# codybloemhard/termdaw

Measured on AMD Instinct MI355X. Metric: offline render Msamples/sec (stereo 48 kHz) + % HBM roofline, 64-vertex graph, higher is better.
Workload: dtype f32; 1 GPU; BASELINE config 2: 64 sampleloop -> 1 normalize, 60 s @48 kHz, bl 1024, 16-bit PCM out; 1 project(s) per GPU per step (project p of the job on rank p mod N, seed offset 64*p); frames_per_project=2880512, projects_per_gpu=1, vertices_per_project=65, normalize=one launch, output=int16 PCM in HBM, parallelism=project p on rank p mod N; one RCCL all-reduce(max) of the 1-entry peak table

## Files before the change

### termdaw_amd/csrc/engine.cpp

```cpp
#include <chrono>

#include "engine.h"
#include "chorus_math.h"
#include "comm.h"
#include "compile.h"
#include "delay_math.h"
#include "devmem.h"
#include "eq_math.h"
#include "midi.h"
#include "sat_math.h"

#include <math.h>
#include <stdlib.h>
#include <string.h>

#include <algorithm>
#include <map>
#include <tuple>
#include <mutex>
#include <condition_variable>
#include <atomic>
#include <thread>
#include <limits>

// ... 242 lines not shown
    const size_t nmax = std::max(nl, nr);
    float *d_lin = nullptr, *d_l = nullptr, *d_r = nullptr, *d_s = nullptr;
    uint8_t* d_raw = nullptr;
    auto cleanup = [&]() {};
    {
        auto up = [](size_t b) { return (b + 255) & ~(size_t)255; };
        const size_t bps_raw = linear ? 0 : (raw_format == PCM_U8 ? 1 : raw_format == PCM_S16 ? 2 : raw_format == PCM_S24 ? 3 : 4);
        const size_t b_lin = up(std::max<size_t>(n_values, 1) * sizeof(float)), b_ch = up(std::max<size_t>(nmax, 1) * sizeof(float));
        const size_t b_raw = up(std::max<size_t>(n_values * bps_raw, 1));
        const size_t need = b_lin + 2 * b_ch + 256 + b_raw;
        if (need > sb->tmp_cap) {
            TD_HIP(hipDeviceSynchronize());
            if (sb->tmp) (void)hipFree(sb->tmp);
            sb->tmp = nullptr;
            sb->tmp_cap = 0;
            TD_HIP(hipMalloc(&sb->tmp, need + need / 2));
            sb->tmp_cap = need + need / 2;
        }
        unsigned char* p = sb->tmp;
        d_lin = reinterpret_cast<float*>(p); p += b_lin;
        d_l = reinterpret_cast<float*>(p); p += b_ch;
        d_r = reinterpret_cast<float*>(p); p += b_ch;
        d_s = reinterpret_cast<float*>(p); p += 256;
        d_raw = p;
    }
    if (linear) {
        TD_HIP(hipMemcpyAsync(d_lin, linear, n_values * sizeof(float), hipMemcpyHostToDevice, st));
    } else {
        const size_t bps = raw_format == PCM_U8 ? 1 : raw_format == PCM_S16 ? 2 : raw_format == PCM_S24 ? 3 : 4;
        TD_HIP(hipMemcpyAsync(d_raw, raw, n_values * bps, hipMemcpyHostToDevice, st));
        launch_pcm_decode(d_raw, d_lin, (uint32_t)n_values, raw_format, st);
    }
    if (pick_loudest) {
        if (channels == 1) {
            launch_sample_split(d_lin, 1, 0, 0, d_l, d_r, (uint32_t)nl, (uint32_t)nr, st);
        } else {
            launch_sample_split(d_lin, 2, 0, 1, d_l, d_r, (uint32_t)nl, (uint32_t)nr, st);
        }
        launch_abs_sum_serial(d_l, (uint32_t)nl, d_s + 4, st);
        launch_abs_sum_serial(d_r, (uint32_t)nr, d_s + 5, st);
        float sums[2];
        TD_HIP(hipMemcpyAsync(sums, d_s + 4, 8, hipMemcpyDeviceToHost, st));
        TD_HIP(hipStreamSynchronize(st));
        const float lm = nl ? sums[0] / (float)nl : 0.0f, rm = nr ? sums[1] / (float)nr : 0.0f;
        const bool take_l = lm > rm;
        const size_t n_take = take_l ? nl : nr;
        if (n_take == 0) { cleanup(); return fail("termdaw_amd: loudest channel is empty"); }
        TD_HIP(hipMemcpyAsync(take_l ? d_r : d_l, take_l ? d_l : d_r, n_take * sizeof(float), hipMemcpyDeviceToDevice, st));
        nl = nr = n_take;
    } else {
        launch_sample_split(d_lin, (uint32_t)channels, src_l, src_r, d_l, d_r, (uint32_t)nl, (uint32_t)nr, st);
    }
    size_t n = nl;
    const float *p_max_l = d_s, *p_max_r = d_s + 1;
    if (method == LM_NORM) {
        launch_absmax(d_l, (uint32_t)nl, d_s, st);
        launch_absmax(d_r, (uint32_t)nr, d_s + 1, st);
    } else if (method == LM_MIX) {
        n = std::min(nl, nr);
        launch_add_planar(d_l, d_r, d_l, (uint32_t)n, st);
        launch_absmax(d_l, (uint32_t)n, d_s, st);
        TD_HIP(hipMemcpyAsync(d_r, d_l, n * sizeof(float), hipMemcpyDeviceToDevice, st));
        p_max_r = d_s;
    } else {
        launch_absmax(d_l, (uint32_t)nl, d_s, st);
        launch_absmax(d_r, (uint32_t)nr, d_s + 1, st);
        launch_absmax(d_s, 2, d_s + 2, st);
        p_max_l = p_max_r = d_s + 2;
    }
    if (nl != nr && method != LM_MIX) { cleanup(); return fail("termdaw_amd: channel lengths differ after load"); }
    if (n == 0) { cleanup(); return fail("TermDaw: Sample::from: l and r have length 0."); }
    SampleEntry e;
    e.len = n;
    e.d = static_cast<float2*>(sb->alloc(0, (n + 16 + (n & 1)) * sizeof(float2)));
    if (!e.d) return 0;
    struct Guard {
        td_samplebank* sb; SampleEntry* e; bool armed = true;
        ~Guard() { if (armed) { sb->release(e->d); sb->release(e->d16); } }
    } guard{sb, &e};
    TD_HIP(hipMemsetAsync(e.d + n, 0, (16 + (n & 1)) * sizeof(float2), st));
    launch_sample_pack(d_l, d_r, p_max_l, p_max_r, e.d, (uint32_t)n, st);
    bool want16 = method != LM_MIX && sr == sb->sample_rate && n >= 1 && n < 0x3FFFFFF0u;
    if (want16) {
        e.d16 = static_cast<uint32_t*>(sb->alloc(1, ((n + 18) & ~(size_t)3) * sizeof(uint32_t)));
        if (!e.d16) return 0;
        TD_HIP(hipMemsetAsync(d_s + 8, 0, sizeof(uint32_t), st));
        launch_sample_pack16(d_l, d_r, e.d16, (uint32_t)n, reinterpret_cast<uint32_t*>(d_s + 8), st);
    }
    float host_s[12] = {0};
    TD_HIP(hipMemcpyAsync(host_s, d_s, sizeof host_s, hipMemcpyDeviceToHost, st));
    TD_HIP(hipStreamSynchronize(st));
    TD_HIP(hipGetLastError());
    if (want16) {
        uint32_t bad;
        memcpy(&bad, &host_s[8], 4);
        const float ml = host_s[p_max_l - d_s], mr = host_s[p_max_r - d_s];
        if (bad) {
            sb->release(e.d16);
            e.d16 = nullptr;
        } else {
            e.scale_l = 1.0f / ml;
            e.scale_r = 1.0f / mr;
        }
    }
    cleanup();
    if (sr != sb->sample_rate) {
        float2* rs = nullptr;
        size_t nout = 0;
        if (!resample_device(e.d, e.len, sr, sb->sample_rate, &rs, &nout, st)) return 0;
        sb->release(e.d);
        e.d = rs;
        if (nout == 0) return fail("termdaw_amd: resampled sample is empty");
        e.len = nout;
    }
    guard.armed = false;
    sb->samples.push_back(e);
    sb->names[name] = sb->samples.size() - 1;
    return 1;
}

}

using namespace tde;

uint64_t td_flowwbank::next_version() {
    static std::atomic<uint64_t> counter{1};
    return counter.fetch_add(1);
}
void td_flowwbank::set_start_indices_to_frame(size_t t_frame, bool do_skip) {
    for (size_t i = 0; i < flowws.size(); ++i) {
        const auto& fl = flowws[i];
        for (size_t j = do_skip ? start_indices[i] : 0; j < fl.size(); ++j) {
            if (frame_of(fl[j]) >= t_frame) {
                start_indices[i] = j;
                break;
            }
        }
    }
}
void td_flowwbank::set_time(size_t t) {
    set_start_indices_to_frame(t, false);
    frame = t;
}
void td_flowwbank::set_time_to_next_block() {
    frame += bl;
    set_start_indices_to_frame(frame, true);
}

namespace tde {
int upload_tables(td_graph* g, TableCache& tc, const Staging& tmp) {
    const size_t bytes = std::max<size_t>(tmp.b.size(), 16);
    if (bytes > tc.cap) {
        TD_HIP(hipStreamSynchronize(g->stream));
        if (tc.d) { (void)hipFree(tc.d); g->device_bytes -= tc.cap; }
        if (tc.h) (void)hipHostFree(tc.h);
        tc.d = tc.h = nullptr;
        tc.cap = 0;
        tc.inflight = false;
        const size_t cap = bytes + bytes / 4 + 256;
        TD_HIP(hipMalloc(&tc.d, cap));
        TD_HIP(hipHostMalloc(&tc.h, cap, hipHostMallocDefault));
        if (!tc.copied) TD_HIP(hipEventCreateWithFlags(&tc.copied, hipEventDisableTiming));
        tc.cap = cap;
        g->device_bytes += cap;
    }
    if (tc.inflight) TD_HIP(hipEventSynchronize(tc.copied));
    tc.inflight = false;
// ... 2710 lines not shown
```

### termdaw_amd/csrc/kernels.h

```cpp
#pragma once
#include <hip/hip_runtime.h>
#include <stdint.h>
#include "adsr_math.h"

namespace tdk {

constexpr int kThreads = 256;
constexpr int kTileFrames = 1024;
constexpr uint32_t kBandMaxSegs = 131072;
constexpr uint32_t kBandMaxS = 1024;

struct PanGain {
    float l_amp, r_amp, gain;
    uint32_t flags;
};

struct InTerm {
    const float2* p;
    uint64_t len;
    uint64_t t0;
    PanGain pg;
    uint32_t kind;
    uint32_t magic;
    float scale_l, scale_r;
};
enum TermMode : uint32_t { TERMS_MIXED = 0, TERMS_ALL_EDGE = 1, TERMS_ALL_LOOP32 = 2, TERMS_ALL_LOOP16 = 3,
                           TERMS_EDGE_FEW = 4,
                           TERMS_ADSR1 = 5,
                           TERMS_WITH_ADSR = 6 };

struct NormState { float max, scan_max; uint32_t violated, ticket; };

struct BandRespParam {
    double ql[8], qh[8];
    double gl, gh;
    double* resp;
};

struct SumDesc {
    const InTerm* ins;
    float2* out;
    float* peaks;
    const NormState* state;
    float* init_copy;
    float init_max;
    uint32_t use_init;
    uint32_t k;
    uint32_t mode;
    uint32_t term_mode;
    uint32_t debug;
    PanGain pg;
    float2* out_q4;
    void* pcm;
    float amplitude;
    uint32_t qmode;
    const BandRespParam* rp;
    unsigned long long* sync;
    uint32_t* host_flag;
};

struct ScaleDesc {
    float2* buf;
    const float* peaks;
    const float* init_copy;
    NormState* state;
    void* pcm;
    float amplitude;
    uint32_t qmode;
    PanGain pg;
    uint32_t pcm_only;
    uint32_t pad[3];
};

struct QuantDesc {
    const float2* in;
    void* pcm;
    float amplitude;
    uint32_t qmode;
};

struct StemDesc {
    InTerm src;
    void* pcm;
    float2* f32;
    uint32_t* peak;
    float amplitude;
    uint32_t qmode;
};

struct LoudDesc {
    const void* pcm;
// ... 470 lines not shown
```

### termdaw_amd/csrc/kernels.hip

```cpp
#include "kernels.h"

#include <algorithm>

namespace tdk {

#define TD_DEV __device__ __forceinline__

TD_DEV float2 epilogue(float2 v, const PanGain& pg) {
    if (pg.flags & 1u) { v.x *= pg.l_amp; v.y *= pg.r_amp; }
    if (pg.flags & 2u) { v.x *= pg.gain;  v.y *= pg.gain;  }
    return v;
}
TD_DEV float4 epilogue4(float4 v, const PanGain& pg) {
    float2 a = epilogue(make_float2(v.x, v.y), pg), b = epilogue(make_float2(v.z, v.w), pg);
    return make_float4(a.x, a.y, b.x, b.y);
}

#define TD_GLOBAL __attribute__((address_space(1)))
typedef float f4v __attribute__((ext_vector_type(4)));
typedef float f2v __attribute__((ext_vector_type(2)));
typedef unsigned int u2v __attribute__((ext_vector_type(2)));
typedef int i4v __attribute__((ext_vector_type(4)));
typedef int i2v __attribute__((ext_vector_type(2)));
TD_DEV float4 gload4(const void* p) { const f4v v = *reinterpret_cast<const f4v TD_GLOBAL*>((const TD_GLOBAL char*)p); return make_float4(v.x, v.y, v.z, v.w); }
// ... 250 lines not shown
#pragma unroll
            for (int u = 0; u < 4; ++u) { const float2* p = ins[j + 4 + u].p; b0[u] = load_pair(p, m0, M); b1[u] = load_pair(p, m1, M); }
#pragma unroll
            for (int u = 0; u < 4; ++u) { acc0 = add4(acc0, a0[u]); acc1 = add4(acc1, a1[u]); }
            if (j + 12 <= k) {
#pragma unroll
                for (int u = 0; u < 4; ++u) { const float2* p = ins[j + 8 + u].p; a0[u] = load_pair(p, m0, M); a1[u] = load_pair(p, m1, M); }
            }
#pragma unroll
            for (int u = 0; u < 4; ++u) { acc0 = add4(acc0, b0[u]); acc1 = add4(acc1, b1[u]); }
        }
        if (j + 4 <= k) {
#pragma unroll
            for (int u = 0; u < 4; ++u) { acc0 = add4(acc0, a0[u]); acc1 = add4(acc1, a1[u]); }
            j += 4;
        }
    }
    for (; j + 4 <= k; j += 4) {
        float4 x0[4], x1[4];
#pragma unroll
        for (int u = 0; u < 4; ++u) {
            if (MODE == TERMS_ALL_EDGE || MODE == TERMS_EDGE_FEW) { const float2* p = ins[j + u].p; x0[u] = load_pair(p, m0, M); x1[u] = load_pair(p, m1, M); }
            else if (MODE == TERMS_ALL_LOOP32) { x0[u] = loop_term_pair(ins, j + u, m0, M); x1[u] = loop_term_pair(ins, j + u, m1, M); }
            else { x0[u] = term_pair(ins, j + u, m0, M); x1[u] = term_pair(ins, j + u, m1, M); }
        }
#pragma unroll
        for (int u = 0; u < 4; ++u) { acc0 = add4(acc0, x0[u]); acc1 = add4(acc1, x1[u]); }
    }
    for (; j < k; ++j) {
        acc0 = add4(acc0, term_pair(ins, j, m0, M));
        acc1 = add4(acc1, term_pair(ins, j, m1, M));
    }
}
typedef unsigned int u4v __attribute__((ext_vector_type(4)));
TD_DEV float2 unpack16(uint32_t w, float sl, float sr) {
    return make_float2((float)(int16_t)(w & 0xFFFFu) * sl, (float)(int16_t)(w >> 16) * sr);
}
typedef unsigned int u4v_u __attribute__((ext_vector_type(4), aligned(4)));
TD_DEV void loop16_quad(const uint32_t* s, uint32_t len, uint32_t idx, uint32_t out[4]) {
    (void)len;
    const uint32_t TD_GLOBAL* g = reinterpret_cast<const uint32_t TD_GLOBAL*>((const TD_GLOBAL char*)s);
    const u4v_u q = *reinterpret_cast<const u4v_u TD_GLOBAL*>(g + idx);
    out[0] = q.x; out[1] = q.y; out[2] = q.z; out[3] = q.w;
}
TD_DEV f2v cvt16(uint32_t w) { f2v v; v.x = (float)(int16_t)(w & 0xFFFFu); v.y = (float)(int16_t)(w >> 16); return v; }
TD_DEV void sum_terms16(TermTab ins, uint32_t k, uint32_t m, uint32_t M, float4& acc0, float4& acc1) {
    f2v c[4];
#pragma unroll
    for (int f = 0; f < 4; ++f) { c[f].x = 0.f; c[f].y = 0.f; }
    auto add_term = [&](uint32_t j, const uint32_t w[4]) {
        f2v sc, am, gn;
        sc.x = ins[j].scale_l; sc.y = ins[j].scale_r;
        am.x = ins[j].pg.l_amp; am.y = ins[j].pg.r_amp;
        gn.x = gn.y = ins[j].pg.gain;
#pragma unroll
        for (int f = 0; f < 4; ++f) {
            f2v v = cvt16(w[f]) * sc;
            v = v * am;
            v = v * gn;
            c[f] = c[f] + v;
        }
    };
    auto gather = [&](uint32_t j, uint32_t w[4]) {
        const uint32_t len = (uint32_t)ins[j].len;
        loop16_quad(reinterpret_cast<const uint32_t*>(ins[j].p), len, barrett_mod((uint32_t)ins[j].t0 + m, len, ins[j].magic), w);
    };
    uint32_t j = 0;
    for (; j + 4 <= k; j += 4) {
        uint32_t w[4][4];
#pragma unroll
        for (int u = 0; u < 4; ++u) gather(j + u, w[u]);
#pragma unroll
        for (int u = 0; u < 4; ++u) add_term(j + u, w[u]);
    }
    for (; j < k; ++j) {
        uint32_t w[4];
        gather(j, w);
        add_term(j, w);
    }
    acc0 = zero_tail(make_float4(c[0].x, c[0].y, c[1].x, c[1].y), m, M);
    acc1 = zero_tail(make_float4(c[2].x, c[2].y, c[3].x, c[3].y), m + 2u, M);
}

TD_DEV uint32_t step256(uint32_t len, uint32_t magic) {
    const uint32_t r = 256u - __umulhi(256u, magic) * len;
    return r >= len ? r - len : r;
}
template <int NQ>
TD_DEV uint32_t quad_frame(uint32_t m, int q) { return NQ == 4 ? m + 256u * (uint32_t)q : m + 4u * (uint32_t)q; }
template <int NQ>
TD_DEV uint32_t pair_frame(uint32_t m, int p) { return quad_frame<NQ>(m, p >> 1) + 2u * (uint32_t)(p & 1); }
template <int NQ>
TD_DEV void sum_terms16w(TermTab ins, uint32_t k, uint32_t m, uint32_t M, float4 acc[2 * NQ]) {
    f2v c[4 * NQ];
#pragma unroll
    for (int f = 0; f < 4 * NQ; ++f) { c[f].x = 0.f; c[f].y = 0.f; }
    auto add_term = [&](uint32_t j, const uint32_t w[4 * NQ]) {
        f2v sc, am, gn;
        sc.x = ins[j].scale_l; sc.y = ins[j].scale_r;
        am.x = ins[j].pg.l_amp; am.y = ins[j].pg.r_amp;
        gn.x = gn.y = ins[j].pg.gain;
#pragma unroll
        for (int f = 0; f < 4 * NQ; ++f) {
            f2v v = cvt16(w[f]) * sc;
            v = v * am;
            v = v * gn;
            c[f] = c[f] + v;
        }
    };
    auto gather = [&](uint32_t j, uint32_t w[4 * NQ]) {
        const uint32_t len = (uint32_t)ins[j].len;
        const uint32_t idx = barrett_mod((uint32_t)ins[j].t0 + m, len, ins[j].magic);
        if (NQ == 4) {
            const uint32_t* p = reinterpret_cast<const uint32_t*>(ins[j].p);
            const uint32_t step = step256(len, ins[j].magic);
            uint32_t i = idx;
#pragma unroll
            for (int q = 0; q < NQ; ++q) {
                loop16_quad(p, len, i, w + 4 * q);
                i += step;
                i = min(i, i - len);
            }
            return;
        }
#pragma unroll
        for (int q = 0; q < NQ; ++q) loop16_quad(reinterpret_cast<const uint32_t*>(ins[j].p), len, idx + 4u * q, w + 4 * q);
    };
    uint32_t j = 0;
    constexpr int B = 4;
    for (; j + B <= k; j += B) {
        uint32_t w[B][4 * NQ];
#pragma unroll
        for (int u = 0; u < B; ++u) gather(j + u, w[u]);
#pragma unroll
        for (int u = 0; u < B; ++u) add_term(j + u, w[u]);
    }
    for (; j < k; ++j) { uint32_t w[4 * NQ]; gather(j, w); add_term(j, w); }
#pragma unroll
    for (int q = 0; q < 2 * NQ; ++q) acc[q] = zero_tail(make_float4(c[2 * q].x, c[2 * q].y, c[2 * q + 1].x, c[2 * q + 1].y), pair_frame<NQ>(m, q), M);
}

template <int NQ>
TD_DEV void sum_terms32w(TermTab ins, uint32_t k, uint32_t m, uint32_t M, float4 acc[2 * NQ]) {
    f4v c[2 * NQ];
#pragma unroll
    for (int q = 0; q < 2 * NQ; ++q) { c[q].x = 0.f; c[q].y = 0.f; c[q].z = 0.f; c[q].w = 0.f; }
    constexpr int B = NQ >= 4 ? 1 : 2;
    auto gather = [&](uint32_t j, f4v x[2 * NQ]) {
        const uint32_t len = (uint32_t)ins[j].len;
        const uint32_t idx = barrett_mod((uint32_t)ins[j].t0 + m, len, ins[j].magic);
        const float2* p = ins[j].p + idx;
#pragma unroll
        for (int q = 0; q < 2 * NQ; ++q) {
            const float4 v = gload4u(p + 2 * q);
            x[q].x = v.x; x[q].y = v.y; x[q].z = v.z; x[q].w = v.w;
        }
    };
    auto add_term = [&](uint32_t j, const f4v x[2 * NQ]) {
        f4v am, gn;
        am.x = am.z = ins[j].pg.l_amp; am.y = am.w = ins[j].pg.r_amp;
        gn.x = gn.y = gn.z = gn.w = ins[j].pg.gain;
#pragma unroll
        for (int q = 0; q < 2 * NQ; ++q) {
            f4v v = x[q] * am;
            v = v * gn;
            c[q] = c[q] + v;
        }
    };
    uint32_t j = 0;
    for (; j + B <= k; j += B) {
        f4v x[B][2 * NQ];
#pragma unroll
        for (int u = 0; u < B; ++u) gather(j + u, x[u]);
#pragma unroll
        for (int u = 0; u < B; ++u) add_term(j + u, x[u]);
    }
    for (; j < k; ++j) { f4v x[2 * NQ]; gather(j, x); add_term(j, x); }
#pragma unroll
    for (int q = 0; q < 2 * NQ; ++q) acc[q] = zero_tail(make_float4(c[q].x, c[q].y, c[q].z, c[q].w), m + 2u * q, M);
}

TD_DEV void sum_inputs_pairs(const InTerm* ins_generic, uint32_t k, uint32_t term_mode, uint32_t m0, uint32_t m1, uint32_t M,
                             float4& a0, float4& a1) {
    const TermTab ins = term_tab(ins_generic);
    a0 = make_float4(0.f, 0.f, 0.f, 0.f);
    a1 = a0;
    if (term_mode == TERMS_ALL_EDGE) sum_terms<TERMS_ALL_EDGE>(ins, k, m0, m1, M, a0, a1);
    else if (term_mode == TERMS_ALL_LOOP32) sum_terms<TERMS_ALL_LOOP32>(ins, k, m0, m1, M, a0, a1);
    else if (term_mode == TERMS_ADSR1) sum_terms<TERMS_ADSR1>(ins, k, m0, m1, M, a0, a1);
    else if (term_mode == TERMS_WITH_ADSR) sum_terms<TERMS_WITH_ADSR>(ins, k, m0, m1, M, a0, a1);
    else sum_terms<TERMS_MIXED>(ins, k, m0, m1, M, a0, a1);
}

TD_DEV float absmax4(float m, float4 v) {
    m = fmaxf(m, fabsf(v.x)); m = fmaxf(m, fabsf(v.y));
    m = fmaxf(m, fabsf(v.z)); m = fmaxf(m, fabsf(v.w));
    return m;
}

template <int TMODE>
__global__ __launch_bounds__(kThreads) void k_sum(const SumDesc* __restrict__ descs, uint32_t M, uint32_t bl,
                                                  uint32_t tiles_per_block) {
    const SumDesc& d = descs[blockIdx.y];
    constexpr bool quad_map = TMODE == TERMS_ALL_LOOP16;
    const uint32_t m0 = blockIdx.x * kTileFrames + (quad_map ? 4 : 2) * threadIdx.x;
    const uint32_t m1 = m0 + (quad_map ? 2 : kTileFrames / 2);
    float4 a0 = make_float4(0.f, 0.f, 0.f, 0.f), a1 = a0;
    if (quad_map) sum_terms16(term_tab(d.ins), d.k, m0, M, a0, a1);
    else sum_terms<TMODE>(term_tab(d.ins), d.k, m0, m1, M, a0, a1);
    if (d.mode == 0) {
        store_pair(d.out, m0, M, epilogue4(a0, d.pg));
        store_pair(d.out, m1, M, epilogue4(a1, d.pg));
        return;
    }
    float spec_init = 0.0f;
    if (d.mode == 3) {
        spec_init = d.use_init ? d.init_max : d.state->max;
        const float r = 1.0f / spec_init;
        const float4 s0 = epilogue4(make_float4(a0.x * r, a0.y * r, a0.z * r, a0.w * r), d.pg);
        const float4 s1 = epilogue4(make_float4(a1.x * r, a1.y * r, a1.z * r, a1.w * r), d.pg);
        if (d.out) {
            store_pair(d.out, m0, M, s0);
// ... 55 lines not shown
            if ((threadIdx.x & 63u) == 63u) {
#pragma unroll
                for (int e = 0; e < 8; ++e) if (!((e & 2) ? want_h : want_l)) rh[e][threadIdx.x >> 6] = 0.0;
            }
            __syncthreads();
            if (threadIdx.x < 16u) {
                const uint32_t blk_in_tile = threadIdx.x >> 2, chain = threadIdx.x & 3u;
                const uint32_t q0 = (blk_in_tile & 1u) * 2u, e = (blk_in_tile >> 1) * 4u + chain;
                const uint32_t blk = blockIdx.x * 4u + blk_in_tile;
                if (blk * 256u < M) rp.resp[4u * blk + chain] = rh[e][q0] + rh[e][q0 + 1u];
            }
        }
        __shared__ float bp[kThreads / 64][2];
        __shared__ uint32_t bc[kThreads / 64][2];
        __shared__ float2 first[4];
        if ((threadIdx.x & 127) == 0) {
            first[(threadIdx.x >> 7)] = make_float2(a0.x, a0.y);
            first[2 + (threadIdx.x >> 7)] = make_float2(a1.x, a1.y);
        }
        __syncthreads();
        const float2 f0 = first[threadIdx.x >> 7], f1 = first[2 + (threadIdx.x >> 7)];
        auto same2 = [](float4 a, float2 f) {
            return __float_as_uint(a.x) == __float_as_uint(f.x) && __float_as_uint(a.y) == __float_as_uint(f.y) &&
                   __float_as_uint(a.z) == __float_as_uint(f.x) && __float_as_uint(a.w) == __float_as_uint(f.y);
        };
        float p0 = m0 < M ? absmax4(0.0f, a0) : 0.0f, p1 = m1 < M ? absmax4(0.0f, a1) : 0.0f;
        const bool c0 = __all((m0 + 1 >= M || same2(a0, f0)) ? 1 : 0) != 0, c1 = __all((m1 + 1 >= M || same2(a1, f1)) ? 1 : 0) != 0;
        p0 = wave_max(p0);
        p1 = wave_max(p1);
        if ((threadIdx.x & 63) == 0) {
            bp[threadIdx.x >> 6][0] = p0; bp[threadIdx.x >> 6][1] = p1;
            bc[threadIdx.x >> 6][0] = c0; bc[threadIdx.x >> 6][1] = c1;
        }
        __syncthreads();
        if (threadIdx.x < 4) {
            const uint32_t half = threadIdx.x & 1u, pair = threadIdx.x >> 1;
            const uint32_t blk = blockIdx.x * 4u + pair * 2u + half;
            const bool cst = bc[2 * half][pair] && bc[2 * half + 1][pair];
            if (blk * 256u < M) d.peaks[blk] = cst ? -1.0f : fmaxf(bp[2 * half][pair], bp[2 * half + 1][pair]);
        }
        return;
    }
    if (blockIdx.x == 0 && threadIdx.x == 0) {
        d.init_copy[0] = d.use_init ? d.init_max : d.state->max;
        d.init_copy[1] = d.state->scan_max;
    }
    const bool spec = d.mode == 3;
    if (tiles_per_block) {
        float pk = 0.0f;
        if (m0 < M) pk = absmax4(pk, a0);
        if (m1 < M) pk = absmax4(pk, a1);
        pk = wave_max(pk);
        __shared__ float wmax[kThreads / 64];
        if ((threadIdx.x & 63) == 0) wmax[threadIdx.x >> 6] = pk;
        __syncthreads();
        if (threadIdx.x == 0) {
            pk = fmaxf(fmaxf(wmax[0], wmax[1]), fmaxf(wmax[2], wmax[3]));
            uint32_t b = blockIdx.x / tiles_per_block;
            if (tiles_per_block == 1) d.peaks[b] = pk;
            else atomicMax(reinterpret_cast<unsigned int*>(d.peaks + b), __float_as_uint(pk));
            if (spec && pk > spec_init) const_cast<NormState*>(d.state)->violated = 1u;
        }
    } else {
        if (spec) {
            const float pk = fmaxf(m0 < M ? absmax4(0.0f, a0) : 0.0f, m1 < M ? absmax4(0.0f, a1) : 0.0f);
            if (pk > spec_init) const_cast<NormState*>(d.state)->violated = 1u;
        }
        const float v[8] = {a0.x, a0.y, a0.z, a0.w, a1.x, a1.y, a1.z, a1.w};
#pragma unroll
        for (int f = 0; f < 4; ++f) {
            uint32_t m = (f < 2 ? m0 : m1) + (f & 1);
            if (m < M) {
                float pk = fmaxf(fmaxf(0.0f, fabsf(v[2 * f])), fabsf(v[2 * f + 1]));
                atomicMax(reinterpret_cast<unsigned int*>(d.peaks + m / bl), __float_as_uint(pk));
            }
        }
    }
}

template <int NQ, bool PACKED = true>
__global__ __launch_bounds__(kThreads) void k_sum16w(const SumDesc* __restrict__ descs, uint32_t M, uint32_t tag) {
    const SumDesc& d = descs[blockIdx.y];
    constexpr int SH = (NQ == 4 && PACKED) ? 4 : 1;
    const uint32_t m = SH == 4 ? blockIdx.x * (kTileFrames * NQ) + (threadIdx.x >> 6) * kTileFrames + 4u * (threadIdx.x & 63u)
                               : blockIdx.x * (kTileFrames * NQ) + 4u * NQ * threadIdx.x;
    const float spec_init_early = d.mode >= 4 ? (d.use_init ? d.init_max : gload1(&d.state->max)) : 0.0f;
    float4 a[2 * NQ];
    if (PACKED) sum_terms16w<NQ>(term_tab(d.ins), d.k, m, M, a);
    else sum_terms32w<NQ>(term_tab(d.ins), d.k, m, M, a);
    if (d.mode == 0) {
#pragma unroll
        for (int q = 0; q < 2 * NQ; ++q) store_pair(d.out, pair_frame<SH>(m, q), M, epilogue4(a[q], d.pg));
        return;
    }
    float pk = 0.0f;
#pragma unroll
    for (int q = 0; q < 2 * NQ; ++q) if (pair_frame<SH>(m, q) < M) pk = absmax4(pk, a[q]);
    float spec_init = 0.0f;
    if (d.mode >= 4) {
        const float init = spec_init_early;
        __shared__ float wm4[kThreads / 64], pm4[kThreads / 64];
        __shared__ uint32_t bad4;
        const uint32_t wave = threadIdx.x >> 6;
        const float pw = wave_max(pk);
        if ((threadIdx.x & 63) == 0) wm4[wave] = pw;
        if (threadIdx.x == 0) bad4 = 0u;
        __syncthreads();
        constexpr uint32_t wpb = 4 / NQ;
        float pb[NQ], T = 0.0f;
#pragma unroll
        for (int b = 0; b < NQ; ++b) {
            float p = wm4[b * wpb];
            for (uint32_t u = 1; u < wpb; ++u) p = fmaxf(p, wm4[b * wpb + u]);
            pb[b] = p;
            T = fmaxf(T, p);
        }
        if (threadIdx.x < (uint32_t)NQ) {
            const uint32_t b = blockIdx.x * NQ + threadIdx.x;
            if (b * kTileFrames < M) d.peaks[b] = threadIdx.x == 0 ? pb[0] : threadIdx.x == 1 ? pb[NQ > 1 ? 1 : 0] : threadIdx.x == 2 ? pb[NQ > 2 ? 2 : 0] : pb[NQ > 3 ? 3 : 0];
        }
        unsigned long long* const sync = d.sync;
        if (threadIdx.x == 0) {
            asm volatile("" ::"v"(init));
            granule_store(sync + blockIdx.x, __float_as_uint(T), tag);
        }
        float pm = 0.0f;
        const bool forced = (d.debug & 1u) != 0u && blockIdx.x != 0u;
        const bool ok = (d.debug & 2u) ? true : !forced && for_lower_granules(sync, blockIdx.x, kScanSpinLimitSum,
                                                      [&pm](uint32_t, uint32_t v) { pm = fmaxf(pm, __uint_as_float(v)); }, tag);
        pm = wave_max(pm);
        if ((threadIdx.x & 63) == 0) pm4[wave] = pm;
        if (!ok) bad4 = 1u;
        __syncthreads();
        float run = fmaxf(fmaxf(fmaxf(pm4[0], pm4[1]), fmaxf(pm4[2], pm4[3])), init);
        float r_mine = 0.0f;
        const uint32_t my_block = wave / wpb;
#pragma unroll
        for (int b = 0; b < NQ; ++b) {
            run = fmaxf(pb[b], run);
            if ((uint32_t)b == my_block) r_mine = 1.0f / run;
        }
        if (threadIdx.x == 0) {
            NormState* st = const_cast<NormState*>(d.state);
            if (bad4) raise_violated(st, d.host_flag);
            else if (blockIdx.x == gridDim.x - 1u) st->max = run;
        }
        spec_init = -1.0f;
#pragma unroll
        for (int q = 0; q < 2 * NQ; ++q) a[q] = epilogue4(make_float4(a[q].x * r_mine, a[q].y * r_mine, a[q].z * r_mine, a[q].w * r_mine), d.pg);
    }
    if (d.mode == 3) {
        spec_init = d.use_init ? d.init_max : d.state->max;
        const float r = 1.0f / spec_init;
#pragma unroll
        for (int q = 0; q < 2 * NQ; ++q) a[q] = epilogue4(make_float4(a[q].x * r, a[q].y * r, a[q].z * r, a[q].w * r), d.pg);
    }
    if (d.mode >= 3) {
        if (d.out) {
#pragma unroll
            for (int q = 0; q < 2 * NQ; ++q) store_pair(d.out, pair_frame<SH>(m, q), M, a[q]);
        }
        if (d.qmode == 1u) {
            uint32_t* o = reinterpret_cast<uint32_t*>(d.pcm);
#pragma unroll
            for (int q = 0; q < NQ; ++q) {
                const uint32_t mm = quad_frame<SH>(m, q);
                if (mm + 3u < M) {
                    const float4 v0 = a[2 * q], v1 = a[2 * q + 1];
                    u4v w;
                    w.x = ((uint32_t)quant16(v0.x, d.amplitude) & 0xFFFFu) | ((uint32_t)quant16(v0.y, d.amplitude) << 16);
                    w.y = ((uint32_t)quant16(v0.z, d.amplitude) & 0xFFFFu) | ((uint32_t)quant16(v0.w, d.amplitude) << 16);
// ... 4604 lines not shown
    }
    return per_cu;
}
int band_scan_resident_capacity(int nf) {
    static int cap_all[kMaxDev][2];
    int* const cap = cap_all[cur_dev()];
    const int i = nf == 16 ? 0 : 1;
    if (cap[i] == 0) {
        int dev = 0;
        hipDeviceProp_t prop;
        const int per_cu = nf == 16 ? band_scan_min_blocks_per_cu<16>() : band_scan_min_blocks_per_cu<8>();
        cap[i] = 1 + ((hipGetDevice(&dev) == hipSuccess && hipGetDeviceProperties(&prop, dev) == hipSuccess) ? per_cu * prop.multiProcessorCount : 0);
    }
    return cap[i] - 1;
}
void launch_band_scan(const BandScanDesc* d, int n, uint32_t frames, uint32_t term_mode, int nf, hipStream_t s) {
    if (!n || !frames) return;
    const uint32_t tile = band_scan_tile_frames(nf), gx = (frames + tile - 1u) / tile;
    switch (term_mode) {
        case TERMS_EDGE_FEW: launch_band_scan_mode<TERMS_EDGE_FEW>(d, n, frames, gx, nf, s); break;
        case TERMS_ALL_EDGE: launch_band_scan_mode<TERMS_ALL_EDGE>(d, n, frames, gx, nf, s); break;
        case TERMS_ADSR1: launch_band_scan_mode<TERMS_ADSR1>(d, n, frames, gx, nf, s); break;
        case TERMS_WITH_ADSR: launch_band_scan_mode<TERMS_WITH_ADSR>(d, n, frames, gx, nf, s); break;
        default: launch_band_scan_mode<TERMS_MIXED>(d, n, frames, gx, nf, s); break;
    }
}
void launch_band_chain(const BandScanDesc* d, int n, uint32_t frames, uint32_t term_mode, bool guarded, hipStream_t s) {
    if (!n || !frames) return;
    const uint32_t tile = band_scan_tile_frames(16), gx = (frames + tile - 1u) / tile;
    void (*k)(const BandScanDesc*, uint32_t, uint32_t) = nullptr;
    switch (term_mode) {
        case TERMS_EDGE_FEW: k = guarded ? k_band_chain<TERMS_EDGE_FEW, true> : k_band_chain<TERMS_EDGE_FEW, false>; break;
        case TERMS_ALL_EDGE: k = guarded ? k_band_chain<TERMS_ALL_EDGE, true> : k_band_chain<TERMS_ALL_EDGE, false>; break;
        case TERMS_ADSR1: k = guarded ? k_band_chain<TERMS_ADSR1, true> : k_band_chain<TERMS_ADSR1, false>; break;
        case TERMS_WITH_ADSR: k = guarded ? k_band_chain<TERMS_WITH_ADSR, true> : k_band_chain<TERMS_WITH_ADSR, false>; break;
        default: k = guarded ? k_band_chain<TERMS_MIXED, true> : k_band_chain<TERMS_MIXED, false>; break;
    }
    if (gx <= (uint32_t)kMaxGridY) {
        hipLaunchKernelGGL(k, dim3((uint32_t)n, gx), dim3(kThreads), 0, s, d, frames, 1u);
    } else {
        for (int o = 0; o < n; o += kMaxGridY)
            hipLaunchKernelGGL(k, dim3(gx, (uint32_t)std::min(n - o, kMaxGridY)), dim3(kThreads), 0, s, d + o, frames, 0u);
    }
}
#undef TD_BATCHED
static inline uint32_t grid_for(uint32_t n) { return max(1u, min((n + kThreads - 1) / kThreads, 2048u)); }
void launch_absmax(const float* v, uint32_t n, float* out, hipStream_t s) {
    (void)hipMemsetAsync(out, 0, sizeof(float), s);
    if (n) hipLaunchKernelGGL(k_absmax_atomic, dim3(grid_for(n)), dim3(kThreads), 0, s, v, n, out);
}
__global__ __launch_bounds__(kThreads) void k_peak_table(const float* const* __restrict__ src, float* __restrict__ table,
                                                         uint32_t n_total, uint32_t n_own, uint32_t first, uint32_t stride) {
    const uint32_t j = blockIdx.x * kThreads + threadIdx.x;
    if (j >= n_total) return;
    float v = 0.0f;
    if (j >= first && (j - first) % stride == 0u && (j - first) / stride < n_own) v = *src[(j - first) / stride];
    table[j] = v;
}
void launch_peak_table(const float* const* src, float* table, uint32_t n_total, uint32_t n_own, uint32_t first, uint32_t stride,
                       hipStream_t s) {
    if (n_total) hipLaunchKernelGGL(k_peak_table, dim3((n_total + kThreads - 1) / kThreads), dim3(kThreads), 0, s, src, table, n_total, n_own, first, stride);
}
void launch_resample(const ResampleDesc& d, hipStream_t s) {
    if (!d.nout) return;
    const uint64_t blocks = (d.nout + kThreads - 1) / kThreads;
    hipLaunchKernelGGL(k_resample, dim3((uint32_t)(blocks < 65535u * 16u ? blocks : 65535u * 16u)), dim3(kThreads), 0, s, d);
}
void launch_pcm_decode(const uint8_t* raw, float* linear, uint32_t n, uint32_t format, hipStream_t s) {
    if (n) hipLaunchKernelGGL(k_pcm_decode, dim3(grid_for(n)), dim3(kThreads), 0, s, raw, linear, n, format);
}
void launch_sample_split(const float* linear, uint32_t channels, uint32_t src_l, uint32_t src_r, float* l, float* r, uint32_t nl,
                         uint32_t nr, hipStream_t s) {
    const uint32_t n = nl > nr ? nl : nr;
    if (n) hipLaunchKernelGGL(k_sample_split, dim3(grid_for(n)), dim3(kThreads), 0, s, linear, channels, src_l, src_r, l, r, nl, nr);
}
void launch_abs_sum_serial(const float* v, uint32_t n, float* out, hipStream_t s) {
    hipLaunchKernelGGL(k_abs_sum_serial, dim3(1), dim3(kThreads), 0, s, v, n, out);
}
void launch_add_planar(const float* a, const float* b, float* out, uint32_t n, hipStream_t s) {
    if (n) hipLaunchKernelGGL(k_add_planar, dim3(grid_for(n)), dim3(kThreads), 0, s, a, b, out, n);
}
__global__ __launch_bounds__(kThreads) void k_sample_pack16(const float* __restrict__ l, const float* __restrict__ r,
                                                            uint32_t* __restrict__ packed, uint32_t n, uint32_t* not_int16) {
    const uint32_t total = (n + 15u + 3u) & ~3u;
    bool bad = false;
    for (uint32_t i = blockIdx.x * kThreads + threadIdx.x; i < total; i += gridDim.x * kThreads) {
        const uint32_t f = i % n;
        const float a = l[f], b = r[f];
        const int ia = (int)fminf(fmaxf(a, -32768.0f), 32767.0f), ib = (int)fminf(fmaxf(b, -32768.0f), 32767.0f);
        bad = bad || (float)ia != a || (float)ib != b;
        packed[i] = ((uint32_t)ia & 0xFFFFu) | ((uint32_t)ib << 16);
    }
    if (__any(bad ? 1 : 0) && (threadIdx.x & 63) == 0) atomicOr(not_int16, 1u);
}
void launch_sample_pack16(const float* l, const float* r, uint32_t* packed, uint32_t n, uint32_t* not_int16, hipStream_t s) {
    if (n) hipLaunchKernelGGL(k_sample_pack16, dim3(grid_for((n + 18u) & ~3u)), dim3(kThreads), 0, s, l, r, packed, n, not_int16);
}
void launch_sample_pack(const float* l, const float* r, const float* max_l, const float* max_r, float2* frames, uint32_t n,
                        hipStream_t s) {
    if (n) hipLaunchKernelGGL(k_sample_pack, dim3(grid_for(n + 15u)), dim3(kThreads), 0, s, l, r, max_l, max_r, frames, n);
}

}
```

Baseline: 49460 Msamples/s.

## Extend packed int16 sample wrap padding so loop gathers skip per-quad modulo

The padded wrap region of packed int16 sample buffers grows from about 16 frames to about 1027 frames. The 16-bit gather can then compute one Barrett modulo per wave-level base frame and read every lane's quads with plain contiguous vector loads at fixed offsets, with no per-quad wrap handling. The base index is made wave-uniform through readfirstlane, which should turn per-lane address math into scalar work. The cost is extra memory for each sample buffer, and correctness depends on the padding being at least as large as the wave's footprint.

```diff
diff --git a/termdaw_amd/csrc/engine.cpp b/termdaw_amd/csrc/engine.cpp
--- a/termdaw_amd/csrc/engine.cpp
+++ b/termdaw_amd/csrc/engine.cpp
@@ -348,7 +348,7 @@
     launch_sample_pack(d_l, d_r, p_max_l, p_max_r, e.d, (uint32_t)n, st);
     bool want16 = method != LM_MIX && sr == sb->sample_rate && n >= 1 && n < 0x3FFFFFF0u;
     if (want16) {
-        e.d16 = static_cast<uint32_t*>(sb->alloc(1, ((n + 18) & ~(size_t)3) * sizeof(uint32_t)));
+        e.d16 = static_cast<uint32_t*>(sb->alloc(1, (size_t)tdk::packed_words((uint32_t)n) * sizeof(uint32_t)));
         if (!e.d16) return 0;
         TD_HIP(hipMemsetAsync(d_s + 8, 0, sizeof(uint32_t), st));
         launch_sample_pack16(d_l, d_r, e.d16, (uint32_t)n, reinterpret_cast<uint32_t*>(d_s + 8), st);
diff --git a/termdaw_amd/csrc/kernels.h b/termdaw_amd/csrc/kernels.h
--- a/termdaw_amd/csrc/kernels.h
+++ b/termdaw_amd/csrc/kernels.h
@@ -7,6 +7,8 @@
 
 constexpr int kThreads = 256;
 constexpr int kTileFrames = 1024;
+constexpr uint32_t kPackWrap = 1023u + 4u;
+constexpr uint32_t packed_words(uint32_t n) { return (n + kPackWrap + 3u) & ~3u; }
 constexpr uint32_t kBandMaxSegs = 131072;
 constexpr uint32_t kBandMaxS = 1024;
 
diff --git a/termdaw_amd/csrc/kernels.hip b/termdaw_amd/csrc/kernels.hip
--- a/termdaw_amd/csrc/kernels.hip
+++ b/termdaw_amd/csrc/kernels.hip
@@ -356,16 +356,12 @@
     acc1 = zero_tail(make_float4(c[2].x, c[2].y, c[3].x, c[3].y), m + 2u, M);
 }
 
-TD_DEV uint32_t step256(uint32_t len, uint32_t magic) {
-    const uint32_t r = 256u - __umulhi(256u, magic) * len;
-    return r >= len ? r - len : r;
-}
 template <int NQ>
 TD_DEV uint32_t quad_frame(uint32_t m, int q) { return NQ == 4 ? m + 256u * (uint32_t)q : m + 4u * (uint32_t)q; }
 template <int NQ>
 TD_DEV uint32_t pair_frame(uint32_t m, int p) { return quad_frame<NQ>(m, p >> 1) + 2u * (uint32_t)(p & 1); }
 template <int NQ>
-TD_DEV void sum_terms16w(TermTab ins, uint32_t k, uint32_t m, uint32_t M, float4 acc[2 * NQ]) {
+TD_DEV uint32_t sum_terms16w(TermTab ins, uint32_t k, uint32_t M, float4 acc[2 * NQ]) {
     f2v c[4 * NQ];
 #pragma unroll
     for (int f = 0; f < 4 * NQ; ++f) { c[f].x = 0.f; c[f].y = 0.f; }
@@ -382,26 +378,24 @@
             c[f] = c[f] + v;
         }
     };
+    const uint32_t mw = blockIdx.x * (kTileFrames * NQ) + (uint32_t)__builtin_amdgcn_readfirstlane((int)(threadIdx.x >> 6)) * (256u * NQ);
+    uint32_t lane_off = (threadIdx.x & 63u) * (NQ == 4 ? 16u : 16u * NQ);
     auto gather = [&](uint32_t j, uint32_t w[4 * NQ]) {
         const uint32_t len = (uint32_t)ins[j].len;
-        const uint32_t idx = barrett_mod((uint32_t)ins[j].t0 + m, len, ins[j].magic);
-        if (NQ == 4) {
-            const uint32_t* p = reinterpret_cast<const uint32_t*>(ins[j].p);
-            const uint32_t step = step256(len, ins[j].magic);
-            uint32_t i = idx;
-#pragma unroll
-            for (int q = 0; q < NQ; ++q) {
-                loop16_quad(p, len, i, w + 4 * q);
-                i += step;
-                i = min(i, i - len);
-            }
-            return;
-        }
-#pragma unroll
-        for (int q = 0; q < NQ; ++q) loop16_quad(reinterpret_cast<const uint32_t*>(ins[j].p), len, idx + 4u * q, w + 4 * q);
+        const uint32_t idx = barrett_mod((uint32_t)ins[j].t0 + mw, len, ins[j].magic);
+        const TD_GLOBAL char* g = (const TD_GLOBAL char*)ins[j].p + 4ull * idx;
+        asm volatile("" : "+v"(lane_off));
+#pragma unroll
+        for (int q = 0; q < NQ; ++q) {
+            const u4v_u v = *reinterpret_cast<const u4v_u TD_GLOBAL*>(g + lane_off + (NQ == 4 ? 1024u : 16u) * (uint32_t)q);
+            w[4 * q] = v.x; w[4 * q + 1] = v.y; w[4 * q + 2] = v.z; w[4 * q + 3] = v.w;
+        }
     };
     uint32_t j = 0;
-    constexpr int B = 4;
+#ifndef TD_SUM16W_BATCH
+#define TD_SUM16W_BATCH 4
+#endif
+    constexpr int B = TD_SUM16W_BATCH;
     for (; j + B <= k; j += B) {
         uint32_t w[B][4 * NQ];
 #pragma unroll
@@ -410,8 +404,10 @@
         for (int u = 0; u < B; ++u) add_term(j + u, w[u]);
     }
     for (; j < k; ++j) { uint32_t w[4 * NQ]; gather(j, w); add_term(j, w); }
+    const uint32_t m = mw + (lane_off >> 2);
 #pragma unroll
     for (int q = 0; q < 2 * NQ; ++q) acc[q] = zero_tail(make_float4(c[2 * q].x, c[2 * q].y, c[2 * q + 1].x, c[2 * q + 1].y), pair_frame<NQ>(m, q), M);
+    return m;
 }
 
 template <int NQ>
@@ -633,11 +629,10 @@
 __global__ __launch_bounds__(kThreads) void k_sum16w(const SumDesc* __restrict__ descs, uint32_t M, uint32_t tag) {
     const SumDesc& d = descs[blockIdx.y];
     constexpr int SH = (NQ == 4 && PACKED) ? 4 : 1;
-    const uint32_t m = SH == 4 ? blockIdx.x * (kTileFrames * NQ) + (threadIdx.x >> 6) * kTileFrames + 4u * (threadIdx.x & 63u)
-                               : blockIdx.x * (kTileFrames * NQ) + 4u * NQ * threadIdx.x;
+    uint32_t m = blockIdx.x * (kTileFrames * NQ) + 4u * NQ * threadIdx.x;
     const float spec_init_early = d.mode >= 4 ? (d.use_init ? d.init_max : gload1(&d.state->max)) : 0.0f;
     float4 a[2 * NQ];
-    if (PACKED) sum_terms16w<NQ>(term_tab(d.ins), d.k, m, M, a);
+    if (PACKED) m = sum_terms16w<NQ>(term_tab(d.ins), d.k, M, a);
     else sum_terms32w<NQ>(term_tab(d.ins), d.k, m, M, a);
     if (d.mode == 0) {
 #pragma unroll
@@ -5408,7 +5403,7 @@
 }
 __global__ __launch_bounds__(kThreads) void k_sample_pack16(const float* __restrict__ l, const float* __restrict__ r,
                                                             uint32_t* __restrict__ packed, uint32_t n, uint32_t* not_int16) {
-    const uint32_t total = (n + 15u + 3u) & ~3u;
+    const uint32_t total = packed_words(n);
     bool bad = false;
     for (uint32_t i = blockIdx.x * kThreads + threadIdx.x; i < total; i += gridDim.x * kThreads) {
         const uint32_t f = i % n;
@@ -5420,7 +5415,7 @@
     if (__any(bad ? 1 : 0) && (threadIdx.x & 63) == 0) atomicOr(not_int16, 1u);
 }
 void launch_sample_pack16(const float* l, const float* r, uint32_t* packed, uint32_t n, uint32_t* not_int16, hipStream_t s) {
-    if (n) hipLaunchKernelGGL(k_sample_pack16, dim3(grid_for((n + 18u) & ~3u)), dim3(kThreads), 0, s, l, r, packed, n, not_int16);
+    if (n) hipLaunchKernelGGL(k_sample_pack16, dim3(grid_for(packed_words(n))), dim3(kThreads), 0, s, l, r, packed, n, not_int16);
 }
 void launch_sample_pack(const float* l, const float* r, const float* max_l, const float* max_r, float2* frames, uint32_t n,
                         hipStream_t s) {
```

Result: slower. 47550 Msamples/s (-3.9%).
